# kabachuha/sd-webui-text2video

Hardware: AMD Instinct MI355X
Metric: denoised frames/sec (UNet+VAE), ModelScope 24f@256x256 (higher is better)
Workload: dtype f16; 1 GPU; ModelScope t2v fp16 (random-init 1.41B UNetSD + VAE decoder), 24 frames @ 256x256, 50 DDIM_Gaussian steps, CFG 9.0 (BASELINE.json configs[1]); one step = one whole video; frames_per_video=24, videos_per_batch=1, layout=single, layout_requested=auto, parallelism=1 GPU: cond+uncond batched as b=2

## Files before the change

### sd-webui-text2video_amd/csrc/attention.hip

```cpp
#include "t2v_kernels.h"

namespace {

struct AttnParams {
  const f16* q; const f16* k; const f16* v; f16* o;
  int nq, nk, heads, b_outer, b_inner;
  long sq_seq, sq_out, sq_in;
  long sk_seq, sk_out, sk_in;
  long so_seq, so_out, so_in;
  float scale_log2;
  int causal;
  int lo_off;
  int alt_from, nk2;
  long sk2_out;
  const f16* k2; const f16* v2;
  const int* tab;
  int nk_max, rows_all;
};

typedef f16 f16x2 __attribute__((ext_vector_type(2)));

template <int D, int NKK>
__device__ __forceinline__ void load_row_frags(f16x8 (&fr)[NKK], const f16* base, int row, const int& nrows, const long& stride, int fhalf) {
#pragma unroll
  for (int kk = 0; kk < NKK; ++kk) {
    const int d0 = kk * 16 + fhalf * 8;
    if (row < nrows && d0 < D)
      fr[kk] = *reinterpret_cast<const f16x8*>(base + (long)row * stride + d0);
    else
      for (int e = 0; e < 8; ++e) fr[kk][e] = (f16)0.f;
  }
}

template <int NB>
__device__ __forceinline__ void mask_keys(f32x16 (&s)[NB], int key0, int key_end, int fhalf) {
#pragma unroll
  for (int T = 0; T < NB; ++T)
#pragma unroll
    for (int r = 0; r < 16; ++r) {
      const int key = key0 + T * 32 + (r & 3) + 8 * (r >> 2) + 4 * fhalf;
      if (key >= key_end) s[T][r] = -INFINITY;
    }
}

struct no_other_sums { __device__ __forceinline__ void operator()(float) const {} };
template <int NB, int NDT, typename Also = no_other_sums>
__device__ __forceinline__ float online_softmax_step(f32x16 (&s)[NB], float scale_log2, float& m_run, float& l_run, f32x16 (&oacc)[NDT],
                                                     Also also = Also()) {
  float mx = -INFINITY;
#pragma unroll
  for (int T = 0; T < NB; ++T)
#pragma unroll
    for (int r = 0; r < 16; ++r) mx = fmaxf(mx, s[T][r]);
  mx = fmaxf(mx, __shfl_xor(mx, 32));
  const float m_tile = mx * scale_log2;
  const bool grow = m_tile - m_run > 8.0f;
  if (__builtin_amdgcn_ballot_w64(grow) != 0) {
    const float alpha = grow ? __builtin_amdgcn_exp2f(m_run - m_tile) : 1.0f;
    l_run *= alpha;
    also(alpha);
#pragma unroll
    for (int d = 0; d < NDT; ++d)
#pragma unroll
      for (int r = 0; r < 16; ++r) oacc[d][r] *= alpha;
    m_run = grow ? m_tile : m_run;
  }
  float psum = 0.f;
  const float neg_m = -m_run;
#pragma unroll
  for (int T = 0; T < NB; ++T)
#pragma unroll
    for (int r = 0; r < 16; ++r) {
      const float pv = __builtin_amdgcn_exp2f(__builtin_fmaf(s[T][r], scale_log2, neg_m));
      s[T][r] = pv;
      psum += pv;
    }
  psum += __shfl_xor(psum, 32);
  l_run += psum;
  return psum;
}

__device__ __forceinline__ f16x8 p_frag(const f32x16& s, int t) {
  f16x8 pf;
#pragma unroll
  for (int e = 0; e < 8; ++e) pf[e] = (f16)s[8 * t + e];
  return pf;
}

template <int NDT>
__device__ __forceinline__ void pv_step(f32x16 (&oacc)[NDT], const unsigned char* img, int pitch, int ofs, const f16x8& pf, int frow) {
#pragma unroll
  for (int d = 0; d < NDT; ++d) {
    const unsigned char* arow = img + (d * 32 + frow) * pitch + ofs;
    const f16x4 lo = *reinterpret_cast<const f16x4*>(arow);
    const f16x4 hi = *reinterpret_cast<const f16x4*>(arow + 16);
    const f16x8 af = {lo[0], lo[1], lo[2], lo[3], hi[0], hi[1], hi[2], hi[3]};
    oacc[d] = __builtin_amdgcn_mfma_f32_32x32x16_f16(af, pf, oacc[d], 0, 0, 0);
  }
}

template <int D, int NKEYS, int NT>
__device__ __forceinline__ void stage_vt(unsigned char* vt, int pitch, const f16* vb, long sk_seq, int key0, int nk, int tid) {
  constexpr int DV = (D + 31) / 32 * 32;
  for (int u = tid; u < (NKEYS / 2) * (DV / 4); u += NT) {
    const int kp = u / (DV / 4), dq = u - kp * (DV / 4);
    const int key = key0 + 2 * kp;
    const bool dok = dq * 4 < D;
    f16x4 a, b;
    if (dok && key < nk) a = *reinterpret_cast<const f16x4*>(vb + (long)key * sk_seq + dq * 4);
    else for (int e = 0; e < 4; ++e) a[e] = (f16)0.f;
    if (dok && key + 1 < nk) b = *reinterpret_cast<const f16x4*>(vb + (long)(key + 1) * sk_seq + dq * 4);
    else for (int e = 0; e < 4; ++e) b[e] = (f16)0.f;
#pragma unroll
    for (int e = 0; e < 4; ++e) {
      f16x2 w = {a[e], b[e]};
      *reinterpret_cast<f16x2*>(vt + (dq * 4 + e) * pitch + kp * 4) = w;
    }
  }
}

template <int D, int NDT>
__device__ __forceinline__ void store_o_hilo(f16* orow, const f32x16 (&oacc)[NDT], float inv, int lo_off, int fhalf) {
  f16* o4 = orow + 4 * fhalf;
#pragma unroll
  for (int d = 0; d < NDT; ++d)
#pragma unroll
    for (int qd = 0; qd < 4; ++qd) {
      const int col = d * 32 + 8 * qd;
      if (col + 4 * fhalf < D) {
        f16x4 o, lo;
#pragma unroll
        for (int r = 0; r < 4; ++r) {
          const float val = oacc[d][4 * qd + r] * inv;
          o[r] = (f16)val;
          lo[r] = (f16)(val - (float)o[r]);
        }
        *reinterpret_cast<f16x4*>(o4 + col) = o;
        if (lo_off) *reinterpret_cast<f16x4*>(o4 + lo_off + col) = lo;
      }
    }
}

template <int NW, int D, int KT = 64, bool TAB = false>
__global__ __launch_bounds__(NW * 64) void attn_kernel(const AttnParams p) {
  constexpr int NT = NW * 64;
  constexpr int NKT = KT / 32;
  constexpr int VT_ROW = KT * 2 + 8;
  constexpr int DK = (D + 15) / 16 * 16;
  constexpr int NKK = DK / 16;
  constexpr int DV = (D + 31) / 32 * 32;
  constexpr int NDT = DV / 32;
  constexpr int KCH = DK / 8;
  constexpr int K_ROW = DK * 2 + 16;
  static_assert(D % 8 == 0, "head_dim must be a multiple of 8");
  __shared__ __attribute__((aligned(16))) unsigned char k_lds[KT * K_ROW];
  __shared__ __attribute__((aligned(16))) unsigned char vt_lds[DV * VT_ROW];

  const int tid = threadIdx.x, lane = tid & 63;
  const int wave = __builtin_amdgcn_readfirstlane(tid >> 6);
  const int head = blockIdx.y;
  const int bo = blockIdx.z / p.b_inner, bi = blockIdx.z % p.b_inner;
  const int q0 = blockIdx.x * (32 * NW) + wave * 32;
  const int frow = lane & 31, fhalf = lane >> 5;

  const f16* qb = p.q + bo * p.sq_out + bi * p.sq_in + head * D;
  int nk;
  const f16 *kb, *vb;
  if constexpr (TAB) {
    const int n = p.tab[2 * bo], first = p.tab[2 * bo + 1];
    nk = (n > 0 && n <= p.nk_max && first >= 0 && first <= p.rows_all - n) ? n : 0;
    const long kv_off = (long)first * p.sk_seq + bi * p.sk_in + head * D;
    kb = p.k + kv_off;
    vb = p.v + kv_off;
  } else {
    const bool alt = p.alt_from > 0 && bo >= p.alt_from;
    nk = alt ? p.nk2 : p.nk;
    const long kv_off = (alt ? (bo - p.alt_from) * p.sk2_out : bo * p.sk_out) + bi * p.sk_in + head * D;
    kb = (alt ? p.k2 : p.k) + kv_off;
    vb = (alt ? p.v2 : p.v) + kv_off;
  }
  f16* ob = p.o + bo * p.so_out + bi * p.so_in + head * D;

  const int qrow = q0 + frow;
  f16x8 qf[NKK];
  load_row_frags<D>(qf, qb, qrow, p.nq, p.sq_seq, fhalf);

  f32x16 oacc[NDT];
#pragma unroll
  for (int d = 0; d < NDT; ++d)
#pragma unroll
    for (int r = 0; r < 16; ++r) oacc[d][r] = 0.f;
  float m_run = -INFINITY, l_run = 0.f;
  const int key_end = p.causal ? min(nk, qrow + 1) : nk;

  for (int kt0 = 0; kt0 < nk; kt0 += KT) {
    __syncthreads();
    for (int u = tid; u < KT * KCH; u += NT) {
      const int row = u / KCH, c = u - row * KCH;
      const int key = kt0 + row;
      f16x8 val;
      if (key < nk && c * 8 < D)
        val = *reinterpret_cast<const f16x8*>(kb + (long)key * p.sk_seq + c * 8);
      else
        for (int e = 0; e < 8; ++e) val[e] = (f16)0.f;
      *reinterpret_cast<f16x8*>(k_lds + row * K_ROW + (c << 4)) = val;
    }
    stage_vt<D, KT, NT>(vt_lds, VT_ROW, vb, p.sk_seq, kt0, nk, tid);
    __syncthreads();

    const bool t1_live = (kt0 + 32) < nk;
    const f32x16 zero16 = {0.f, 0.f, 0.f, 0.f, 0.f, 0.f, 0.f, 0.f, 0.f, 0.f, 0.f, 0.f, 0.f, 0.f, 0.f, 0.f};
    f32x16 s[NKT];
#pragma unroll
    for (int T = 0; T < NKT; ++T) {
      s[T] = zero16;
      if (T == 1 && !t1_live) continue;
      const int row = T * 32 + frow;
#pragma unroll
      for (int kk = 0; kk < NKK; ++kk) {
        const f16x8 kf = *reinterpret_cast<const f16x8*>(k_lds + row * K_ROW + ((kk * 2 + fhalf) << 4));
        s[T] = __builtin_amdgcn_mfma_f32_32x32x16_f16(kf, qf[kk], kk == 0 ? zero16 : s[T], 0, 0, 0);
      }
    }
    if (kt0 + KT > nk || (p.causal && kt0 + KT - 1 > q0)) mask_keys(s, kt0, key_end, fhalf);
    online_softmax_step(s, p.scale_log2, m_run, l_run, oacc);

#pragma unroll
    for (int T = 0; T < NKT; ++T) {
      if (T == 1 && !t1_live) continue;
#pragma unroll
      for (int t = 0; t < 2; ++t)
        pv_step(oacc, vt_lds, VT_ROW, (T * 32 + t * 16 + 4 * fhalf) * 2, p_frag(s[T], t), frow);
    }
  }

  if (qrow < p.nq) store_o_hilo<D>(ob + (long)qrow * p.so_seq, oacc, 1.0f / l_run, p.lo_off, fhalf);
}

__device__ __attribute__((aligned(256))) unsigned char attn_zero_page[256];

__global__ __launch_bounds__(256) void vt_transpose_kernel(const AttnParams p, f16* vt, int n_pad) {
  __shared__ f16 tile[64][66];
  const int tid = threadIdx.x;
  const int head = blockIdx.y, bo = blockIdx.z / p.b_inner, bi = blockIdx.z % p.b_inner;
  const int k0 = blockIdx.x * 64;
  const f16* vb = p.v + bo * p.sk_out + bi * p.sk_in + head * 64;
#pragma unroll
  for (int i = 0; i < 2; ++i) {
    const int u = tid + i * 256, key = u >> 3, c = u & 7;
    f16x8 val;
    if (k0 + key < p.nk) val = *reinterpret_cast<const f16x8*>(vb + (long)(k0 + key) * p.sk_seq + c * 8);
    else for (int e = 0; e < 8; ++e) val[e] = (f16)0.f;
#pragma unroll
    for (int e = 0; e < 8; ++e) tile[key][c * 8 + e] = val[e];
  }
  __syncthreads();
  f16* out = vt + ((long)blockIdx.z * p.heads + head) * 64 * n_pad + k0;
#pragma unroll
  for (int i = 0; i < 2; ++i) {
    const int u = tid + i * 256, d = u >> 3, c = u & 7;
    f16x8 val;
#pragma unroll
    for (int e = 0; e < 8; ++e) {
      const int g = c >> 1, f = c & 1;
      val[e] = tile[16 * g + 4 * f + (e & 3) + 8 * (e >> 2)][d];
    }
    *reinterpret_cast<f16x8*>(out + (long)d * n_pad + c * 8) = val;
  }
}

template <int NW>
__global__ __launch_bounds__(NW * 64, 4) void attn2_kernel(const AttnParams p, const f16* __restrict__ vt, int n_pad) {
  constexpr int D = 64, KT = 64, NKK = 4, NDT = 2, NKT = 2;
  constexpr int PIECES = 16, PPW = PIECES / NW;
  static_assert(PIECES % NW == 0, "pieces must divide over the waves");
  __shared__ __attribute__((aligned(16))) unsigned char smem[2 * 16384];

  const int tid = threadIdx.x, lane = tid & 63;
  const int wave = __builtin_amdgcn_readfirstlane(tid >> 6);
  const int head = blockIdx.y;
  const int bo = blockIdx.z / p.b_inner, bi = blockIdx.z % p.b_inner;
  const int q0 = blockIdx.x * (32 * NW) + wave * 32;
  const int frow = lane & 31, fhalf = lane >> 5;

  const f16* qb = p.q + bo * p.sq_out + bi * p.sq_in + head * D;
  const f16* kb = p.k + bo * p.sk_out + bi * p.sk_in + head * D;
  const f16* vtb = vt + ((long)blockIdx.z * p.heads + head) * 64 * n_pad;
  f16* ob = p.o + bo * p.so_out + bi * p.so_in + head * D;

  const int qrow = q0 + frow;
  f16x8 qf[NKK];
  load_row_frags<D>(qf, qb, qrow, p.nq, p.sq_seq, fhalf);
  f32x16 oacc[NDT];
#pragma unroll
  for (int d = 0; d < NDT; ++d)
#pragma unroll
    for (int r = 0; r < 16; ++r) oacc[d][r] = 0.f;
  float m_run = -INFINITY, l_run = 0.f;

  const int lrow = lane >> 3, pch = lane & 7;
  const f16* src0[PPW];
#pragma unroll
  for (int i = 0; i < PPW; ++i) {
    const int j = wave + NW * i, row = 8 * (j & 7) + lrow, lc = pch ^ ((row >> 1) & 7);
    src0[i] = j < 8 ? kb + (long)row * p.sk_seq + lc * 8 : vtb + (long)row * n_pad + lc * 8;
  }
  auto stage = [&](int t, int buf) {
#pragma unroll
    for (int i = 0; i < PPW; ++i) {
      const int j = wave + NW * i;
      const f16* src = src0[i] + (long)t * (j < 8 ? (long)KT * p.sk_seq : (long)KT);
      if (j < 8 && t * KT + 8 * (j & 7) + lrow >= p.nk) src = reinterpret_cast<const f16*>(attn_zero_page);
      __builtin_amdgcn_global_load_lds((const __attribute__((address_space(1))) void*)src,
                                       (__attribute__((address_space(3))) void*)(smem + buf * 16384 + (j >> 3) * 8192 + (j & 7) * 1024), 16, 0, 0);
    }
  };
  const int nt = (p.nk + KT - 1) / KT;
  const int sw = ((frow >> 1) & 7);
  stage(0, 0);
  for (int t = 0; t < nt; ++t) {
    const int kt0 = t * KT;
    asm volatile("s_waitcnt vmcnt(0)" ::: "memory");
    __builtin_amdgcn_s_barrier();
    asm volatile("" ::: "memory");
    if (t + 1 < nt) stage(t + 1, (t + 1) & 1);
    const unsigned char* kl = smem + (t & 1) * 16384;
    const unsigned char* vl = kl + 8192;
    const bool t1_live = (kt0 + 32) < p.nk;
    const f32x16 zero16 = {0.f, 0.f, 0.f, 0.f, 0.f, 0.f, 0.f, 0.f, 0.f, 0.f, 0.f, 0.f, 0.f, 0.f, 0.f, 0.f};
    f32x16 s[NKT];
#pragma unroll
    for (int T = 0; T < NKT; ++T) {
      s[T] = zero16;
      if (T == 1 && !t1_live) continue;
#pragma unroll
      for (int kk = 0; kk < NKK; ++kk) {
        const f16x8 kf = *reinterpret_cast<const f16x8*>(kl + (T * 32 + frow) * 128 + (((kk * 2 + fhalf) ^ sw) << 4));
        s[T] = __builtin_amdgcn_mfma_f32_32x32x16_f16(kf, qf[kk], kk == 0 ? zero16 : s[T], 0, 0, 0);
      }
    }
    if (kt0 + KT > p.nk) mask_keys(s, kt0, p.nk, fhalf);
    online_softmax_step(s, p.scale_log2, m_run, l_run, oacc);
#pragma unroll
    for (int T = 0; T < NKT; ++T) {
      if (T == 1 && !t1_live) continue;
#pragma unroll
      for (int u = 0; u < 2; ++u) {
        const f16x8 pf = p_frag(s[T], u);
#pragma unroll
        for (int d = 0; d < NDT; ++d) {
          const f16x8 vf = *reinterpret_cast<const f16x8*>(vl + (d * 32 + frow) * 128 + (((4 * T + 2 * u + fhalf) ^ sw) << 4));
          oacc[d] = __builtin_amdgcn_mfma_f32_32x32x16_f16(vf, pf, oacc[d], 0, 0, 0);
        }
      }
    }
  }
  if (qrow < p.nq) store_o_hilo<D>(ob + (long)qrow * p.so_seq, oacc, 1.0f / l_run, p.lo_off, fhalf);
}

struct SeqAttnParams {
  const f16* q; const f16* k; const f16* v; f16* o;
  const float* ek; const float* ev;
  int T, D, heads, b_inner, R, lds_per_wave;
  int Tq, q_off;
  long n_items;
  long sq_seq, sq_out, sq_in;
  long sk_seq, sk_out, sk_in;
  long so_seq, so_out, so_in;
  float scale;
  int lo_off;
};

__device__ __forceinline__ f32x8 ld_f32x8(const float* p) {
  const f32x4 a = *reinterpret_cast<const f32x4*>(p), b = *reinterpret_cast<const f32x4*>(p + 4);
  f32x8 r = {a[0], a[1], a[2], a[3], b[0], b[1], b[2], b[3]};
  return r;
}

template <int TB, bool REL>
__global__ __launch_bounds__(256) void seqattn_kernel(const SeqAttnParams p) {
  extern __shared__ __attribute__((aligned(16))) unsigned char ssm[];
  const int lane = threadIdx.x & 63;
  const int wave = __builtin_amdgcn_readfirstlane(threadIdx.x >> 6);
  const long item = (long)blockIdx.x * 4 + wave;
  const bool live = item < p.n_items;
  const int T = p.T, D = p.D, d8 = D >> 3;
  const int DP = D * 2 + 16;
  unsigned char* qs = ssm + (size_t)wave * p.lds_per_wave;
  unsigned char* ks = qs + T * DP;
  unsigned char* vs = ks + T * DP;
  float* ps = reinterpret_cast<float*>(vs + T * DP);
  const int head = live ? (int)(item % p.heads) : 0;
  const long pos = live ? item / p.heads : 0;
  const long bo = pos / p.b_inner, bi = pos % p.b_inner;
  const f16* qb = p.q + bo * p.sq_out + bi * p.sq_in + head * D;
  const f16* kb = p.k + bo * p.sk_out + bi * p.sk_in + head * D;
  const f16* vb = p.v + bo * p.sk_out + bi * p.sk_in + head * D;
  f16* ob = p.o + bo * p.so_out + bi * p.so_in + head * D;
  const int Tq = p.Tq;
  if (live) {
    for (int u = lane; u < T * d8; u += 64) {
      const int t = u / d8, c = u - t * d8;
      if (t < Tq) *reinterpret_cast<f16x8*>(qs + t * DP + c * 16) = *reinterpret_cast<const f16x8*>(qb + (long)t * p.sq_seq + c * 8);
      *reinterpret_cast<f16x8*>(ks + t * DP + c * 16) = *reinterpret_cast<const f16x8*>(kb + (long)t * p.sk_seq + c * 8);
      *reinterpret_cast<f16x8*>(vs + t * DP + c * 16) = *reinterpret_cast<const f16x8*>(vb + (long)t * p.sk_seq + c * 8);
    }
  }
  __syncthreads();
  if (live) {
    const int ti = lane >> 3, sj = lane & 7;
    float acc[TB][TB];
#pragma unroll
    for (int a = 0; a < TB; ++a)
#pragma unroll
      for (int b = 0; b < TB; ++b) acc[a][b] = 0.f;
    int rrow[2 * TB - 1];
    if (REL) {
#pragma unroll
      for (int e = 0; e < 2 * TB - 1; ++e) {
        int dlt = 8 * (e - (TB - 1)) + sj - ti - p.q_off;
        dlt = dlt < -p.R ? -p.R : (dlt > p.R ? p.R : dlt);
        rrow[e] = (dlt + p.R) * D;
      }
    }
    for (int c = 0; c < d8; ++c) {
      f16x8 qv[TB], kv[TB];
#pragma unroll
      for (int a = 0; a < TB; ++a) {
        const int t = ti + 8 * a;
        if (t < Tq) qv[a] = *reinterpret_cast<const f16x8*>(qs + t * DP + c * 16);
        else for (int j = 0; j < 8; ++j) qv[a][j] = (f16)0.f;
      }
#pragma unroll
      for (int b = 0; b < TB; ++b) {
        const int sx = sj + 8 * b;
        if (sx < T) kv[b] = *reinterpret_cast<const f16x8*>(ks + sx * DP + c * 16);
        else for (int j = 0; j < 8; ++j) kv[b][j] = (f16)0.f;
      }
      if (REL) {
        f32x8 er[2 * TB - 1];
#pragma unroll
        for (int e = 0; e < 2 * TB - 1; ++e) er[e] = ld_f32x8(p.ek + rrow[e] + c * 8);
#pragma unroll
        for (int a = 0; a < TB; ++a)
#pragma unroll
          for (int b = 0; b < TB; ++b)
#pragma unroll
            for (int j = 0; j < 8; ++j) acc[a][b] += (float)qv[a][j] * ((float)kv[b][j] + er[b - a + TB - 1][j]);
      } else {
#pragma unroll
        for (int a = 0; a < TB; ++a)
#pragma unroll
          for (int b = 0; b < TB; ++b)
#pragma unroll
            for (int j = 0; j < 8; ++j) acc[a][b] += (float)qv[a][j] * (float)kv[b][j];
      }
    }
#pragma unroll
    for (int a = 0; a < TB; ++a) {
      const int t = ti + 8 * a;
      float mx = -INFINITY;
#pragma unroll
      for (int b = 0; b < TB; ++b) {
        acc[a][b] = (sj + 8 * b < T) ? acc[a][b] * p.scale : -INFINITY;
        mx = fmaxf(mx, acc[a][b]);
      }
      mx = fmaxf(mx, __shfl_xor(mx, 1)); mx = fmaxf(mx, __shfl_xor(mx, 2)); mx = fmaxf(mx, __shfl_xor(mx, 4));
      float sum = 0.f;
#pragma unroll
      for (int b = 0; b < TB; ++b) { acc[a][b] = __expf(acc[a][b] - mx); sum += acc[a][b]; }
      sum += __shfl_xor(sum, 1); sum += __shfl_xor(sum, 2); sum += __shfl_xor(sum, 4);
      const float inv = 1.0f / sum;
      if (t < Tq) {
#pragma unroll
        for (int b = 0; b < TB; ++b)
          if (sj + 8 * b < T) ps[t * (T + 1) + sj + 8 * b] = acc[a][b] * inv;
      }
    }
  }
  __syncthreads();
  if (live) {
    for (int u = lane; u < Tq * d8; u += 64) {
      const int t = u / d8, c = u - t * d8;
      f32x8 o;
#pragma unroll
      for (int j = 0; j < 8; ++j) o[j] = 0.f;
      for (int sx = 0; sx < T; ++sx) {
        const float pv = ps[t * (T + 1) + sx];
        const f16x8 vv = *reinterpret_cast<const f16x8*>(vs + sx * DP + c * 16);
        if (REL) {
          int dlt = sx - t - p.q_off;
          dlt = dlt < -p.R ? -p.R : (dlt > p.R ? p.R : dlt);
          const f32x8 e = ld_f32x8(p.ev + (long)(dlt + p.R) * D + c * 8);
#pragma unroll
          for (int j = 0; j < 8; ++j) o[j] += pv * ((float)vv[j] + e[j]);
        } else {
#pragma unroll
          for (int j = 0; j < 8; ++j) o[j] += pv * (float)vv[j];
        }
      }
      f16x8 oh, ol;
#pragma unroll
      for (int j = 0; j < 8; ++j) { oh[j] = (f16)o[j]; ol[j] = (f16)(o[j] - (float)oh[j]); }
      *reinterpret_cast<f16x8*>(ob + (long)t * p.so_seq + c * 8) = oh;
      if (p.lo_off) *reinterpret_cast<f16x8*>(ob + p.lo_off + (long)t * p.so_seq + c * 8) = ol;
    }
  }
}


struct RelMfmaParams {
  SeqAttnParams a;
  int jbase;
  int nblk;
};

template <int D>
__global__ __launch_bounds__(256) void relpos_mfma_kernel(const RelMfmaParams pp) {
  const SeqAttnParams& p = pp.a;
  constexpr int DK = (D + 15) / 16 * 16, NKK = DK / 16;
  constexpr int DV = (D + 31) / 32 * 32, NDT = DV / 32;
  constexpr int EK_PITCH = DK * 2 + 16;
  constexpr int EV_PITCH = 64 * 2 + 8;
  constexpr int VT_PITCH = 32 * 2 + 8;
  constexpr int QE_PITCH = 65;
  constexpr int P_PITCH = 128;
  constexpr int WAVE_BYTES = DV * VT_PITCH + 32 * QE_PITCH * 4 + 32 * P_PITCH * 2;
  extern __shared__ __attribute__((aligned(16))) unsigned char ssm[];
  unsigned char* ekl = ssm;
  unsigned char* evt = ssm + 64 * EK_PITCH;
  const int tid = threadIdx.x, lane = tid & 63;
  const int wave = __builtin_amdgcn_readfirstlane(tid >> 6);
  unsigned char* wbase = ssm + 64 * EK_PITCH + DV * EV_PITCH + wave * WAVE_BYTES;
  unsigned char* vt = wbase;
  float* qeb = reinterpret_cast<float*>(wbase + DV * VT_PITCH);
  f16* pb = reinterpret_cast<f16*>(wbase + DV * VT_PITCH + 32 * QE_PITCH * 4);
  const int T = p.T, R = p.R;
  const int nrows = 2 * R + 1;
  for (int u = tid; u < 64 * (DK / 8); u += 256) {
// ... 242 lines not shown
  constexpr int DK = (D + 15) / 16 * 16, DV = (D + 31) / 32 * 32;
  constexpr int lds = 32 * (DK * 2 + 16) + DV * (32 * 2 + 8) + 4 * (DV * (16 * 2 + 8) + 16 * 33 * 4 + 16 * 64 * 2);
  static_assert(lds <= 160 * 1024, "LDS budget");
  Rel16Params pp;
  pp.a = p;
  pp.ek16 = ek16;
  pp.evt16 = evt16;
  auto kern = relpos16_kernel<D>;
  static t2v_device_flags attr_set;
  {
    const hipError_t e = t2v_set_dynamic_lds(reinterpret_cast<const void*>(kern), lds, attr_set, s);
    if (e != hipSuccess) return e;
  }
  const int per_cu = (160 * 1024 / lds) < 4 ? (160 * 1024 / lds) : 4;
  const long want = (p.n_items + 3) / 4, hold = (long)t2v_num_cus(s) * per_cu;
  hipLaunchKernelGGL(kern, dim3((unsigned)(want < hold ? want : hold)), dim3(256), lds, s, pp);
  return hipGetLastError();
}

struct RelLongParams {
  SeqAttnParams a;
  const f16* ek16;
  const f16* evt16;
  int nc;
  int nqb;
  long n_units;
};

template <int D>
__global__ __launch_bounds__(256) void relpos_long_kernel(const RelLongParams pp) {
  const SeqAttnParams& p = pp.a;
  constexpr int DK = (D + 15) / 16 * 16, NKK = DK / 16;
  constexpr int DV = (D + 31) / 32 * 32, NDT = DV / 32;
  constexpr int VT_PITCH = 32 * 2 + 8;
  constexpr int QE_PITCH = 35;
  constexpr int P_PITCH = 40;
  constexpr int WAVE_BYTES = DV * VT_PITCH + 64 * QE_PITCH * 4;
  static_assert(WAVE_BYTES % 16 == 0 && (DV * VT_PITCH) % 16 == 0 && 32 * P_PITCH * 2 <= 64 * QE_PITCH * 4, "LDS carve-up");
  extern __shared__ __attribute__((aligned(16))) unsigned char ssm[];
  const int lane = threadIdx.x & 63;
  const int wave = __builtin_amdgcn_readfirstlane(threadIdx.x >> 6);
  const long unit = (long)blockIdx.x * 4 + wave;
  if (unit >= pp.n_units) return;
  unsigned char* vt = ssm + wave * WAVE_BYTES;
  float* qeb = reinterpret_cast<float*>(vt + DV * VT_PITCH);
  f16* pb = reinterpret_cast<f16*>(qeb);
  const long item = unit / pp.nqb;
  const int t0 = (int)(unit - item * pp.nqb) * 32;
  const int head = (int)(item % p.heads);
  const long pos = item / p.heads;
  const long bo = pos / p.b_inner, bi = pos % p.b_inner;
  const f16* qb = p.q + bo * p.sq_out + bi * p.sq_in + head * D;
  const f16* kb = p.k + bo * p.sk_out + bi * p.sk_in + head * D;
  const f16* vb = p.v + bo * p.sk_out + bi * p.sk_in + head * D;
  f16* ob = p.o + bo * p.so_out + bi * p.so_in + head * D;
  const int T = p.T, R = p.R, Tq = p.Tq, nc = pp.nc;
  const int t0a = t0 + p.q_off;
  const int frow = lane & 31, fhalf = lane >> 5;
  const int tq = t0 + frow;
  const f32x16 zero16 = {0.f, 0.f, 0.f, 0.f, 0.f, 0.f, 0.f, 0.f, 0.f, 0.f, 0.f, 0.f, 0.f, 0.f, 0.f, 0.f};
  f16x8 qf[NKK];
  load_row_frags<D>(qf, qb, tq, Tq, p.sq_seq, fhalf);
  float qe_lo, qe_hi;
  {
    const f16* erow = pp.ek16 + (long)(frow < 16 ? 0 : 2 * R) * DK;
    f32x16 qe = zero16;
#pragma unroll
    for (int kk = 0; kk < NKK; ++kk)
      qe = __builtin_amdgcn_mfma_f32_32x32x16_f16(*reinterpret_cast<const f16x8*>(erow + kk * 16 + fhalf * 8), qf[kk], qe, 0, 0, 0);
    qe_lo = qe[0];
    qe_hi = qe[8];
  }
  f32x16 oacc[NDT];
#pragma unroll
  for (int d = 0; d < NDT; ++d) oacc[d] = zero16;
  float m_run = -INFINITY, l_run = 0.f, w_lo = 0.f, w_hi = 0.f;
  bool any_edge = false;
  const float sl2 = p.scale * 1.44269504088896340736f;
  for (int s0 = 0; s0 < T; s0 += 32) {
    const int dmin = s0 - (t0a + 31), dmax = s0 + 31 - t0a;
    const int edge = dmin >= R ? 1 : (dmax <= -R ? -1 : 0);
    any_edge |= edge != 0;
    stage_vt<D, 32, 64>(vt, VT_PITCH, vb, p.sk_seq, s0, T, lane);
    f32x16 sc[1] = {zero16};
    {
      const int key = s0 + frow;
#pragma unroll
      for (int kk = 0; kk < NKK; ++kk) {
        const int d0 = kk * 16 + fhalf * 8;
        f16x8 kf;
        if (key < T && d0 < D) kf = *reinterpret_cast<const f16x8*>(kb + (long)key * p.sk_seq + d0);
        else for (int e = 0; e < 8; ++e) kf[e] = (f16)0.f;
        sc[0] = __builtin_amdgcn_mfma_f32_32x32x16_f16(kf, qf[kk], sc[0], 0, 0, 0);
      }
    }
    const int jb = s0 - t0a - 31 + R;
    if (edge == 0) {
#pragma unroll
      for (int blk = 0; blk < 2; ++blk) {
        int row = jb + blk * 32 + frow;
        row = row < 0 ? 0 : (row > 2 * R ? 2 * R : row);
        const f16* erow = pp.ek16 + (long)row * DK;
        f32x16 qe = zero16;
#pragma unroll
        for (int kk = 0; kk < NKK; ++kk)
          qe = __builtin_amdgcn_mfma_f32_32x32x16_f16(*reinterpret_cast<const f16x8*>(erow + kk * 16 + fhalf * 8), qf[kk], qe, 0, 0, 0);
#pragma unroll
        for (int g = 0; g < 4; ++g)
#pragma unroll
          for (int e = 0; e < 4; ++e) qeb[(blk * 32 + 8 * g + 4 * fhalf + e) * QE_PITCH + frow] = qe[4 * g + e];
      }
    }
    __builtin_amdgcn_fence(__ATOMIC_RELEASE, "wavefront");
#pragma unroll
    for (int r = 0; r < 16; ++r) {
      const int kl = (r & 3) + 8 * (r >> 2) + 4 * fhalf;
      const float rel = edge > 0 ? qe_hi : (edge < 0 ? qe_lo : qeb[(kl - frow + 31) * QE_PITCH + frow]);
      sc[0][r] = (s0 + kl < T) ? sc[0][r] + rel : -INFINITY;
    }
    const float psum = online_softmax_step(sc, sl2, m_run, l_run, oacc, [&](float alpha) { w_lo *= alpha; w_hi *= alpha; });
    if (edge > 0) w_hi += psum;
    if (edge < 0) w_lo += psum;
#pragma unroll
    for (int t2 = 0; t2 < 2; ++t2) pv_step(oacc, vt, VT_PITCH, (t2 * 16 + 4 * fhalf) * 2, p_frag(sc[0], t2), frow);
    if (edge == 0) {
#pragma unroll
      for (int g = 0; g < 4; ++g) {
        const f16x4 pw = {(f16)sc[0][4 * g], (f16)sc[0][4 * g + 1], (f16)sc[0][4 * g + 2], (f16)sc[0][4 * g + 3]};
        *reinterpret_cast<f16x4*>(pb + frow * P_PITCH + 8 * g + 4 * fhalf) = pw;
      }
      __builtin_amdgcn_fence(__ATOMIC_RELEASE, "wavefront");
      const int cb = jb + T2V_RELPOS_LONG_PADL;
      const int dl = cb & 7, c0 = cb - dl;
      const int nst = (dl + 62) / 16 + 1;
      for (int u = 0; u < nst; ++u) {
        f16x8 pf;
#pragma unroll
        for (int e = 0; e < 8; ++e) {
          const int kl = 16 * u + 4 * fhalf + (e & 3) + 8 * (e >> 2) - dl + frow - 31;
          pf[e] = (kl >= 0 && kl < 32) ? pb[frow * P_PITCH + kl] : (f16)0.f;
        }
        const int cofs = c0 + 16 * u + 4 * fhalf;
#pragma unroll
        for (int d = 0; d < NDT; ++d) {
          const f16* erow = pp.evt16 + (long)(d * 32 + frow) * nc + cofs;
          const f16x4 lo = *reinterpret_cast<const f16x4*>(erow);
          const f16x4 hi = *reinterpret_cast<const f16x4*>(erow + 8);
          const f16x8 ef = {lo[0], lo[1], lo[2], lo[3], hi[0], hi[1], hi[2], hi[3]};
          oacc[d] = __builtin_amdgcn_mfma_f32_32x32x16_f16(ef, pf, oacc[d], 0, 0, 0);
        }
      }
    }
    __builtin_amdgcn_fence(__ATOMIC_RELEASE, "wavefront");
  }
  if (any_edge) {
#pragma unroll
    for (int d = 0; d < NDT; ++d)
#pragma unroll
      for (int r = 0; r < 16; ++r) {
        const f16* ecol = pp.evt16 + (long)(d * 32 + (r & 3) + 8 * (r >> 2) + 4 * fhalf) * nc + T2V_RELPOS_LONG_PADL;
        oacc[d][r] += w_lo * (float)ecol[0] + w_hi * (float)ecol[2 * R];
      }
  }
  if (tq < Tq) store_o_hilo<D>(ob + (long)tq * p.so_seq, oacc, 1.0f / l_run, p.lo_off, fhalf);
}

template <int D>
hipError_t launch_relpos_long(const SeqAttnParams& p, const f16* ek16, const f16* evt16, hipStream_t s) {
  constexpr int DV = (D + 31) / 32 * 32;
  constexpr int lds = 4 * (DV * (32 * 2 + 8) + 64 * 35 * 4);
  static_assert(lds <= 160 * 1024, "LDS budget");
  RelLongParams pp;
  pp.a = p;
  pp.ek16 = ek16;
  pp.evt16 = evt16;
  pp.nc = T2V_RELPOS_LONG_COLS(p.R);
  pp.nqb = (p.Tq + 31) / 32;
  pp.n_units = p.n_items * pp.nqb;
  auto kern = relpos_long_kernel<D>;
  static t2v_device_flags attr_set;
  {
    const hipError_t e = t2v_set_dynamic_lds(reinterpret_cast<const void*>(kern), lds, attr_set, s);
    if (e != hipSuccess) return e;
  }
  hipLaunchKernelGGL(kern, dim3((unsigned)((pp.n_units + 3) / 4)), dim3(256), lds, s, pp);
  return hipGetLastError();
}

template <bool REL>
hipError_t launch_seqattn(const t2v_op& op, hipStream_t s) {
  SeqAttnParams p;
  p.q = reinterpret_cast<const f16*>(op.p[0]); p.k = reinterpret_cast<const f16*>(op.p[1]); p.v = reinterpret_cast<const f16*>(op.p[2]);
  p.o = reinterpret_cast<f16*>(op.p[3]);
  p.ek = reinterpret_cast<const float*>(op.p[4]);
  p.ev = reinterpret_cast<const float*>(op.p[5]);
  p.Tq = op.i[0]; p.T = op.i[1]; p.heads = op.i[2]; p.b_inner = op.i[4]; p.D = op.i[14] > 0 ? op.i[14] : 64; p.R = op.i[15];
  p.q_off = op.i[16];
  p.n_items = (long)op.i[3] * op.i[4] * p.heads;
  p.sq_seq = op.i[5]; p.sq_out = op.i[6]; p.sq_in = op.i[7];
  p.sk_seq = op.i[8]; p.sk_out = op.i[9]; p.sk_in = op.i[10];
  p.so_seq = op.i[11]; p.so_out = op.i[12]; p.so_in = op.i[13];
  p.scale = op.f[0];
  p.lo_off = REL ? op.i[18] : 0;
  if (REL && op.i[17] == 3) {
    if (p.T <= 0 || p.T > T2V_RELPOS_MAX_FRAMES || p.Tq <= 0 || p.q_off < 0 || p.q_off + p.Tq > p.T || p.R < 0 || p.n_items <= 0 ||
        !(p.scale > 0.f) || op.p[6] == 0 || op.p[7] == 0)
      return hipErrorInvalidValue;
    const f16* ek16 = reinterpret_cast<const f16*>(op.p[6]);
    const f16* evt16 = reinterpret_cast<const f16*>(op.p[7]);
    switch (p.D) {
      case 40: return launch_relpos_long<40>(p, ek16, evt16, s);
      case 64: return launch_relpos_long<64>(p, ek16, evt16, s);
      case 80: return launch_relpos_long<80>(p, ek16, evt16, s);
      case 160: return launch_relpos_long<160>(p, ek16, evt16, s);
      default: return hipErrorInvalidValue;
    }
  }
  if (p.T <= 0 || p.T > 32 || p.Tq <= 0 || p.q_off < 0 || p.q_off + p.Tq > p.T || p.D <= 0 || p.D % 8 != 0 || p.D > 160 || p.n_items <= 0)
    return hipErrorInvalidValue;
  if (REL && (p.R < 0 || p.ek == nullptr || p.ev == nullptr)) return hipErrorInvalidValue;
  if (REL && op.i[17] == 2 && op.p[6] != 0 && op.p[7] != 0 && p.Tq == p.T && p.q_off == 0 && p.T <= 16 && p.R >= p.T - 1 && p.scale > 0.f) {
    const f16* ek16 = reinterpret_cast<const f16*>(op.p[6]);
    const f16* evt16 = reinterpret_cast<const f16*>(op.p[7]);
    switch (p.D) {
      case 40: return launch_relpos16<40>(p, ek16, evt16, s);
      case 64: return launch_relpos16<64>(p, ek16, evt16, s);
      case 80: return launch_relpos16<80>(p, ek16, evt16, s);
      case 160: return launch_relpos16<160>(p, ek16, evt16, s);
      default: break;
    }
  }
  if (REL && op.i[17] == 1 && p.Tq == p.T && p.q_off == 0 && p.R >= p.T - 1 && p.R <= 31 && p.scale > 0.f) {
    {
      switch (p.D) {
        case 40: return launch_relpos_mfma<40>(p, s);
        case 64: return launch_relpos_mfma<64>(p, s);
        case 80: return launch_relpos_mfma<80>(p, s);
        case 160: return launch_relpos_mfma<160>(p, s);
        default: break;
      }
    }
  }
  p.lds_per_wave = (3 * p.T * (p.D * 2 + 16) + p.T * (p.T + 1) * 4 + 15) / 16 * 16;
  const int lds = 4 * p.lds_per_wave;
  const dim3 grid((unsigned)((p.n_items + 3) / 4));
  const int tb = (p.T + 7) / 8;
  auto go = [&](auto kern) -> hipError_t {
    static t2v_device_flags attr_set;
    {
      const hipError_t e = t2v_set_dynamic_lds(reinterpret_cast<const void*>(kern), 160 * 1024, attr_set, s);
      if (e != hipSuccess) return e;
    }
    hipLaunchKernelGGL(kern, grid, dim3(256), lds, s, p);
    return hipGetLastError();
  };
  switch (tb) {
    case 1: return go(seqattn_kernel<1, REL>);
    case 2: return go(seqattn_kernel<2, REL>);
    case 3: return go(seqattn_kernel<3, REL>);
    default: return go(seqattn_kernel<4, REL>);
  }
}

__global__ __launch_bounds__(256) void softmax_rows_kernel(const float* in, f16* out, int rows, int cols,
                                                           int ld_in, int ld_out, float scale) {
  __shared__ float red[4];
  const int row = blockIdx.x;
  if (row >= rows) return;
  const float* x = in + (size_t)row * ld_in;
  const int tid = threadIdx.x, lane = tid & 63, wave = tid >> 6;
  float mx = -INFINITY;
  for (int c = tid; c < cols; c += 256) mx = fmaxf(mx, x[c] * scale);
  for (int o = 32; o > 0; o >>= 1) mx = fmaxf(mx, __shfl_xor(mx, o));
  if (lane == 0) red[wave] = mx;
  __syncthreads();
  mx = fmaxf(fmaxf(red[0], red[1]), fmaxf(red[2], red[3]));
  __syncthreads();
  float sum = 0.f;
  for (int c = tid; c < cols; c += 256) sum += __expf(x[c] * scale - mx);
  for (int o = 32; o > 0; o >>= 1) sum += __shfl_xor(sum, o);
  if (lane == 0) red[wave] = sum;
  __syncthreads();
  sum = red[0] + red[1] + red[2] + red[3];
  const float inv = 1.0f / sum;
  f16* y = out + (size_t)row * ld_out;
  for (int c = tid; c < cols; c += 256) y[c] = (f16)(__expf(x[c] * scale - mx) * inv);
}

template <int D>
void launch_attn(const AttnParams& p, int nbatch, hipStream_t s) {
  const bool small = p.nq <= 32;
  const dim3 g1(1, p.heads, nbatch), g4((p.nq + 127) / 128, p.heads, nbatch);
  if (p.tab != nullptr) {
    if (small && p.nk_max <= 32) hipLaunchKernelGGL((attn_kernel<1, D, 32, true>), g1, dim3(64), 0, s, p);
    else if (small) hipLaunchKernelGGL((attn_kernel<1, D, 64, true>), g1, dim3(64), 0, s, p);
    else hipLaunchKernelGGL((attn_kernel<4, D, 64, true>), g4, dim3(256), 0, s, p);
    return;
  }
  if (small && (p.nk > p.nk2 ? p.nk : p.nk2) <= 32) hipLaunchKernelGGL((attn_kernel<1, D, 32>), g1, dim3(64), 0, s, p);
  else if (small) hipLaunchKernelGGL((attn_kernel<1, D, 64>), g1, dim3(64), 0, s, p);
  else hipLaunchKernelGGL((attn_kernel<4, D, 64>), g4, dim3(256), 0, s, p);
}

}

t2v_attention_class t2v_attention_classify(const t2v_op& op) {
  const int d = op.i[14] > 0 ? op.i[14] : 64;
  auto is = [&](t2v_attention_form form) { return t2v_attention_class{form, d, op.i[18] == 4 ? 4 : 8, nullptr}; };
  auto bad = [&](const char* why) { return t2v_attention_class{T2V_ATTN_MALFORMED, d, 0, why}; };
  if (op.i[0] <= 0 || op.i[1] <= 0 || op.i[2] <= 0 || op.i[3] <= 0 || op.i[4] <= 0) return bad("empty attention");
  if (d != 40 && d != 64 && d != 80 && d != 160) return bad("attention head_dim must be 40, 64, 80 or 160");
  for (int k = 5; k <= 13; ++k)
    if (op.i[k] < 0) return bad("negative attention stride");
  if (op.i[15] != 0 && op.i[0] != op.i[1]) return bad("causal attention needs nq == nk");
  if (op.i[16] < 0) return bad("negative low-order output offset");
  if (!(op.f[0] > 0.f)) return bad("attention scale must be > 0");
  if (op.p[0] == 0 || op.p[1] == 0 || op.p[2] == 0 || op.p[3] == 0) return bad("null attention pointer");
  if (op.p[6] != 0 && (d != 64 || op.i[15] != 0 || op.i[17] < op.i[1] || op.i[17] % 64 != 0 || (op.i[18] != 0 && op.i[18] != 4 && op.i[18] != 8)))
    return bad("attention with a V^T scratch (p[6]): head_dim 64, not causal, i[17] = keys padded to a multiple of 64, i[18] = 0 | 4 | 8 waves");
  if (op.i[19] != 0) {
    if (op.i[19] < 0 || op.i[19] >= op.i[3] || op.i[20] <= 0 || op.i[21] < 0 || op.p[4] == 0 || op.p[5] == 0)
      return bad("attention second role: 0 < i[19] < batch_outer, i[20] keys > 0, sample stride i[21] >= 0, K / V bases p[4], p[5]");
    if (op.i[15] != 0 || op.p[6] != 0) return bad("attention second role: not for causal launches or the V^T scratch path");
  }
  if (op.i[22] != 0 || op.i[23] != 0 || op.i[24] != 0) {
    if (op.p[7] == 0) return bad("attention per-sample table: null table p[7]");
    if (op.i[22] != op.i[3] || op.i[23] <= 0 || op.i[24] < op.i[23])
      return bad("attention per-sample table: i[22] rows == batch_outer, i[23] largest key count > 0, i[24] K / V rows spanned >= i[23]");
    if (op.i[19] != 0 || op.i[20] != 0 || op.i[21] != 0 || op.p[4] != 0 || op.p[5] != 0) return bad("attention per-sample table: not together with the second role (i[19..21], p[4], p[5])");
    if (op.i[15] != 0) return bad("attention per-sample table: not for causal launches");
    if (op.p[6] != 0) return bad("attention per-sample table: not for the V^T scratch path (p[6])");
    return is(T2V_ATTN_TABLE);
  }
  if (op.p[7] != 0) return bad("attention table p[7] without its fields i[22..24]");
  return is(op.p[6] != 0 ? T2V_ATTN_VT : op.i[19] != 0 ? T2V_ATTN_SECOND_ROLE : T2V_ATTN_PLAIN);
}

hipError_t t2v_launch_attention(const t2v_op& op, hipStream_t s) {
  const t2v_attention_class c = t2v_attention_classify(op);
  AttnParams p;
  p.q = reinterpret_cast<const f16*>(op.p[0]); p.k = reinterpret_cast<const f16*>(op.p[1]); p.v = reinterpret_cast<const f16*>(op.p[2]);
  p.o = reinterpret_cast<f16*>(op.p[3]);
  p.nq = op.i[0]; p.nk = op.i[1]; p.heads = op.i[2]; p.b_outer = op.i[3]; p.b_inner = op.i[4];
  p.sq_seq = op.i[5]; p.sq_out = op.i[6]; p.sq_in = op.i[7];
  p.sk_seq = op.i[8]; p.sk_out = op.i[9]; p.sk_in = op.i[10];
  p.so_seq = op.i[11]; p.so_out = op.i[12]; p.so_in = op.i[13];
  p.scale_log2 = op.f[0] * 1.44269504088896340736f;
  p.causal = op.i[15] != 0;
  p.lo_off = op.i[16];
  p.alt_from = op.i[19]; p.nk2 = c.form == T2V_ATTN_SECOND_ROLE ? op.i[20] : 0; p.sk2_out = op.i[21];
  p.k2 = reinterpret_cast<const f16*>(op.p[4]); p.v2 = reinterpret_cast<const f16*>(op.p[5]);
  p.tab = c.form == T2V_ATTN_TABLE ? reinterpret_cast<const int*>(op.p[7]) : nullptr;
  p.nk_max = op.i[23]; p.rows_all = op.i[24];
  const int nbatch = p.b_outer * p.b_inner;
  switch (c.form) {
    case T2V_ATTN_MALFORMED: return hipErrorInvalidValue;
    case T2V_ATTN_VT: {
      f16* vt = reinterpret_cast<f16*>(op.p[6]);
      const int n_pad = op.i[17];
      hipLaunchKernelGGL(vt_transpose_kernel, dim3(n_pad / 64, p.heads, nbatch), dim3(256), 0, s, p, vt, n_pad);
      if (c.vt_waves == 4) hipLaunchKernelGGL((attn2_kernel<4>), dim3((p.nq + 127) / 128, p.heads, nbatch), dim3(256), 0, s, p, vt, n_pad);
      else hipLaunchKernelGGL((attn2_kernel<8>), dim3((p.nq + 255) / 256, p.heads, nbatch), dim3(512), 0, s, p, vt, n_pad);
      break;
    }
    default:
      if (c.head_dim == 40) launch_attn<40>(p, nbatch, s);
      else if (c.head_dim == 64) launch_attn<64>(p, nbatch, s);
      else if (c.head_dim == 80) launch_attn<80>(p, nbatch, s);
      else launch_attn<160>(p, nbatch, s);
  }
  return hipGetLastError();
}

hipError_t t2v_launch_relpos_attention(const t2v_op& op, hipStream_t s) { return launch_seqattn<true>(op, s); }

hipError_t t2v_launch_softmax(const t2v_op& op, hipStream_t s) {
  hipLaunchKernelGGL(softmax_rows_kernel, dim3(op.i[0]), dim3(256), 0, s,
                     reinterpret_cast<const float*>(op.p[0]), reinterpret_cast<f16*>(op.p[1]), op.i[0],
                     op.i[1], op.i[2], op.i[3], op.f[0]);
  return hipGetLastError();
}
```

Measured before the change: 18.11 frames/s.

## Add persistent cross-attention kernel that stages K/V once per head and loops query blocks

Adds a persistent xattn kernel for non-causal attention with at most 96 keys and shared K/V across the inner batch. Each block stages all keys and transposed V into LDS once per (batch, head) pair. Its four waves then loop over many query blocks, prefetching the next Q fragments while computing the current block. The grid is sized from occupancy capacity so K/V loads are not repeated across many small blocks. The path is on by default through an env flag, adds LDS pressure for large head dims, and may lose parallelism when there are few query blocks.

Measured after the change: 18.08 frames/s. Within noise of the previous version (-0.2%).

```diff
diff --git a/sd-webui-text2video_amd/csrc/attention.hip b/sd-webui-text2video_amd/csrc/attention.hip
--- a/sd-webui-text2video_amd/csrc/attention.hip
+++ b/sd-webui-text2video_amd/csrc/attention.hip
@@ -1,4 +1,7 @@
 #include "t2v_kernels.h"
+
+#include <cstdlib>
+#include <cstring>
 
 namespace {
 
@@ -235,6 +238,117 @@
   }
 
   if (qrow < p.nq) store_o_hilo<D>(ob + (long)qrow * p.so_seq, oacc, 1.0f / l_run, p.lo_off, fhalf);
+}
+
+constexpr int XATTN_KEYS = 96;
+
+template <int D>
+__global__ __launch_bounds__(256) void xattn_kernel(const AttnParams p, const int wpp) {
+  constexpr int NT = 256, NW = 4;
+  constexpr int VT_ROW = XATTN_KEYS * 2 + 8;
+  constexpr int DK = (D + 15) / 16 * 16;
+  constexpr int NKK = DK / 16;
+  constexpr int DV = (D + 31) / 32 * 32;
+  constexpr int NDT = DV / 32;
+  constexpr int KCH = DK / 8;
+  constexpr int K_ROW = DK * 2 + 16;
+  static_assert(D % 8 == 0, "head_dim must be a multiple of 8");
+  __shared__ __attribute__((aligned(16))) unsigned char k_lds[XATTN_KEYS * K_ROW];
+  __shared__ __attribute__((aligned(16))) unsigned char vt_lds[DV * VT_ROW];
+
+  const int tid = threadIdx.x, lane = tid & 63;
+  const int wave = __builtin_amdgcn_readfirstlane(tid >> 6);
+  const int pair = blockIdx.x / wpp, part = blockIdx.x - pair * wpp;
+  const int bo = pair / p.heads, head = pair - bo * p.heads;
+  const int frow = lane & 31, fhalf = lane >> 5;
+
+  const bool alt = p.alt_from > 0 && bo >= p.alt_from;
+  const int nk = alt ? p.nk2 : p.nk;
+  const long kv_off = (alt ? (bo - p.alt_from) * p.sk2_out : bo * p.sk_out) + head * D;
+  const f16* kb = (alt ? p.k2 : p.k) + kv_off;
+  const f16* vb = (alt ? p.v2 : p.v) + kv_off;
+
+  for (int u = tid; u < XATTN_KEYS * KCH; u += NT) {
+    const int key = u / KCH, c = u - key * KCH;
+    f16x8 val;
+    if (key < nk && c * 8 < D)
+      val = *reinterpret_cast<const f16x8*>(kb + (long)key * p.sk_seq + c * 8);
+    else
+      for (int e = 0; e < 8; ++e) val[e] = (f16)0.f;
+    *reinterpret_cast<f16x8*>(k_lds + key * K_ROW + (c << 4)) = val;
+  }
+  stage_vt<D, XATTN_KEYS, NT>(vt_lds, VT_ROW, vb, p.sk_seq, 0, nk, tid);
+  __syncthreads();
+
+  const int nqb = (p.nq + 31) / 32;
+  const int n_items = p.b_inner * nqb;
+  const int step = wpp * NW;
+  const bool t1_live = 32 < nk, tile1 = 64 < nk;
+  const f32x16 zero16 = {0.f, 0.f, 0.f, 0.f, 0.f, 0.f, 0.f, 0.f, 0.f, 0.f, 0.f, 0.f, 0.f, 0.f, 0.f, 0.f};
+
+  int item = part * NW + wave;
+  f16x8 qf[NKK], qn[NKK];
+  if (item < n_items) {
+    const int bi = item / nqb, qb = item - bi * nqb;
+    load_row_frags<D>(qf, p.q + bo * p.sq_out + bi * p.sq_in + head * D, qb * 32 + frow, p.nq, p.sq_seq, fhalf);
+  }
+  while (item < n_items) {
+    const int bi = item / nqb, qb = item - bi * nqb;
+    const int qrow = qb * 32 + frow;
+    const int next = item + step;
+    if (next < n_items) {
+      const int nbi = next / nqb, nqblk = next - nbi * nqb;
+      load_row_frags<D>(qn, p.q + bo * p.sq_out + nbi * p.sq_in + head * D, nqblk * 32 + frow, p.nq, p.sq_seq, fhalf);
+    }
+
+    f32x16 oacc[NDT];
+#pragma unroll
+    for (int d = 0; d < NDT; ++d) oacc[d] = zero16;
+    float m_run = -INFINITY, l_run = 0.f;
+
+    {
+      f32x16 s[2];
+#pragma unroll
+      for (int T = 0; T < 2; ++T) {
+        s[T] = zero16;
+        if (T == 1 && !t1_live) continue;
+        const int row = T * 32 + frow;
+#pragma unroll
+        for (int kk = 0; kk < NKK; ++kk) {
+          const f16x8 kf = *reinterpret_cast<const f16x8*>(k_lds + row * K_ROW + ((kk * 2 + fhalf) << 4));
+          s[T] = __builtin_amdgcn_mfma_f32_32x32x16_f16(kf, qf[kk], kk == 0 ? zero16 : s[T], 0, 0, 0);
+        }
+      }
+      if (64 > nk) mask_keys(s, 0, nk, fhalf);
+      online_softmax_step(s, p.scale_log2, m_run, l_run, oacc);
+#pragma unroll
+      for (int T = 0; T < 2; ++T) {
+        if (T == 1 && !t1_live) continue;
+#pragma unroll
+        for (int t = 0; t < 2; ++t)
+          pv_step(oacc, vt_lds, VT_ROW, (T * 32 + t * 16 + 4 * fhalf) * 2, p_frag(s[T], t), frow);
+      }
+    }
+    if (tile1) {
+      f32x16 s[1];
+#pragma unroll
+      for (int kk = 0; kk < NKK; ++kk) {
+        const f16x8 kf = *reinterpret_cast<const f16x8*>(k_lds + (64 + frow) * K_ROW + ((kk * 2 + fhalf) << 4));
+        s[0] = __builtin_amdgcn_mfma_f32_32x32x16_f16(kf, qf[kk], kk == 0 ? zero16 : s[0], 0, 0, 0);
+      }
+      mask_keys(s, 64, nk, fhalf);
+      online_softmax_step(s, p.scale_log2, m_run, l_run, oacc);
+#pragma unroll
+      for (int t = 0; t < 2; ++t)
+        pv_step(oacc, vt_lds, VT_ROW, (64 + t * 16 + 4 * fhalf) * 2, p_frag(s[0], t), frow);
+    }
+
+    if (qrow < p.nq)
+      store_o_hilo<D>(p.o + bo * p.so_out + bi * p.so_in + head * D + (long)qrow * p.so_seq, oacc, 1.0f / l_run, p.lo_off, fhalf);
+#pragma unroll
+    for (int kk = 0; kk < NKK; ++kk) qf[kk] = qn[kk];
+    item = next;
+  }
 }
 
 __device__ __attribute__((aligned(256))) unsigned char attn_zero_page[256];
@@ -1083,6 +1197,40 @@
   else hipLaunchKernelGGL((attn_kernel<4, D, 64>), g4, dim3(256), 0, s, p);
 }
 
+constexpr int XATTN_PERSIST_DEFAULT = 1;
+bool xattn_persist_enabled() {
+  static int mode = -1;
+  if (mode < 0) {
+    const char* e = getenv("T2V_XATTN_PERSIST");
+    mode = e != nullptr ? (strcmp(e, "0") != 0 ? 1 : 0) : XATTN_PERSIST_DEFAULT;
+  }
+  return mode == 1;
+}
+
+bool xattn_selects(const t2v_attention_class& c, const AttnParams& p) {
+  if (c.form != T2V_ATTN_PLAIN && c.form != T2V_ATTN_SECOND_ROLE) return false;
+  if (p.causal || p.sk_in != 0) return false;
+  return (p.nk > p.nk2 ? p.nk : p.nk2) <= XATTN_KEYS;
+}
+
+template <int D>
+hipError_t launch_xattn(const AttnParams& p, hipStream_t s) {
+  auto kern = xattn_kernel<D>;
+  static int occ[T2V_MAX_DEVICES] = {};
+  const long hold = t2v_grid_capacity(reinterpret_cast<const void*>(kern), 256, 0, s, occ);
+  if (hold <= 0) return hipErrorInvalidConfiguration;
+  const long npairs = (long)p.b_outer * p.heads;
+  const long slots = ((long)p.b_inner * ((p.nq + 31) / 32) + 3) / 4;
+  long wpp = hold / npairs;
+  if (wpp < 1) wpp = 1;
+  if (wpp > slots) wpp = slots;
+  const long rounds = (slots + wpp - 1) / wpp;
+  wpp = (slots + rounds - 1) / rounds;
+  if (npairs * wpp > 0x7fffffffL) return hipErrorInvalidValue;
+  hipLaunchKernelGGL(kern, dim3((unsigned)(npairs * wpp)), dim3(256), 0, s, p, (int)wpp);
+  return hipGetLastError();
+}
+
 }
 
 t2v_attention_class t2v_attention_classify(const t2v_op& op) {
@@ -1145,6 +1293,12 @@
       break;
     }
     default:
+      if (xattn_persist_enabled() && xattn_selects(c, p)) {
+        if (c.head_dim == 40) return launch_xattn<40>(p, s);
+        if (c.head_dim == 64) return launch_xattn<64>(p, s);
+        if (c.head_dim == 80) return launch_xattn<80>(p, s);
+        return launch_xattn<160>(p, s);
+      }
       if (c.head_dim == 40) launch_attn<40>(p, nbatch, s);
       else if (c.head_dim == 64) launch_attn<64>(p, nbatch, s);
       else if (c.head_dim == 80) launch_attn<80>(p, nbatch, s);
```
